# swoonge/SC-A-LOAM

Hardware: AMD Instinct MI355X
Metric: scans/sec (feat-extract + scan-to-map ICP + SC loop search), KITTI HDL-64 (higher is better)
Workload: dtype f32 points / f64 pose algebra

## Files before the change

### sc-a-loam_amd/csrc/common.hpp

```cpp
#pragma once
#include <hip/hip_runtime.h>
#include <hip/hip_ext.h>
#include <cstdio>
#include <cstdarg>
#include <cstring>
#include <string>
#include <vector>
#include <utility>
#include <mutex>
#include "../../include/scaloam_hip.h"
#include "batch.hpp"

namespace scal {
constexpr unsigned EV_DEVICE_ONLY = hipEventDisableTiming | hipEventDisableSystemFence;


void set_error(const char* fmt, ...);

#define SCAL_HIP(expr)                                                                         \
    do {                                                                                       \
        hipError_t _e = (expr);                                                                \
        if (_e != hipSuccess) {                                                                \
            ::scal::set_error("%s failed: %s (%s:%d)", #expr, hipGetErrorString(_e), __FILE__, __LINE__); \
            return SCAL_E_HIP;                                                                 \
        }                                                                                      \
    } while (0)

#define SCAL_TRY(expr)           \
    do {                         \
        int _rc = (expr);        \
        if (_rc != SCAL_OK) return _rc; \
    } while (0)

int select_device(int device);
enum class StreamLayout { Shared, PerStage };
enum { STAGE_FEATURES = 0, STAGE_SC = 1, STAGE_ODOM = 3, STAGE_MAP = 4, STAGE_MAP_PREFETCH = 2, STAGE_SC_FILTER = 5 };
int stage_lane(StreamLayout layout, int stage);
StreamLayout default_stream_layout();
int acquire_stream(int device, hipStream_t* out, int lane = 0);
void release_stream(int device, int lane = 0);
int odom_create(const scal_odom_config* cfg, StreamLayout layout, scal_odom_t** out);
int map_create(const scal_map_config* cfg, StreamLayout layout, scal_map_t** out);
int sc_create(const scal_sc_config* cfg, StreamLayout layout, scal_sc_t** out);
int icp_create_on_lane(const scal_icp_config* cfg, int lane, scal_icp_t** out);
int refine_create_on_lane(const scal_refine_config* cfg, int lane, scal_refine_t** out);
int posegraph_create_on_lane(const scal_posegraph_config* cfg, int lane, scal_posegraph_t** out);
struct ScFilterOut {
    const float *x, *y, *z, *w;
    const int* d_n;
    int cap;
};
int sc_insert_features_then(scal_sc_t* ctx, scal_features_t* feat, int (*after)(void* user, hipStream_t s, const ScFilterOut& ds), void* user);

int sc_make_cloud_device(scal_sc_t* ctx, const float* d_x, const float* d_y, const float* d_z, const int* d_n, int n_max, double* d_desc);

struct LaneStream {
    hipStream_t s = nullptr;
    int device = 0, lane = 0;
    LaneStream() = default;
    LaneStream(LaneStream&& o) noexcept { *this = std::move(o); }
    LaneStream& operator=(LaneStream&& o) noexcept {
        release();
        std::swap(s, o.s);
        device = o.device, lane = o.lane;
        return *this;
    }
    ~LaneStream() { release(); }
    operator hipStream_t() const { return s; }
    int acquire(int dev, int ln) {
        release();
        device = dev, lane = ln;
        return acquire_stream(dev, &s, ln);
    }
    void release() {
        if (s) release_stream(device, lane);
        s = nullptr;
// ... 147 lines not shown
```

### sc-a-loam_amd/csrc/mapping.hip

```cpp
#include "common.hpp"
#include <mutex>
#include <atomic>
#include "device_utils.hpp"
#include "voxel_dev.hpp"
#include "radix_sort.hpp"
#include "lm_host.hpp"
#include "features_dev.hpp"
#include <cmath>
#include <cstdlib>
#include <algorithm>
#include <deque>

namespace scal {

constexpr int CW = 21, CH = 21, CD = 11;
constexpr int GX = 250, GY = 250, GZ = 150;
constexpr int GCELLS = GX * GY * GZ;
constexpr unsigned long long MAP_NOMERGE = 127ull;

struct MapParams {
    int cenW, cenH, cenD;
    int cI, cJ, cK;
    int ox, oy, oz;
    float inv_line, inv_plane;
// ... 1089 lines not shown
__device__ __forceinline__ void k_merge_write_body(const MergeArgs& a, MapState* S, MapCounters* C, const MergeTail& t) {
    merge_write_body(a, S, C);
    if (!t.fused) return;
    if (static_cast<int>(blockIdx.x) >= MERGE_WRITE_GRID && S->pose_seq == t.seq) {
        const int i = (blockIdx.x - MERGE_WRITE_GRID) * 256 + threadIdx.x;
        if (i < min(*t.d_nfull, t.full_cap)) {
            double x7[7];
#pragma unroll
            for (int k = 0; k < 7; ++k) x7[k] = t.st->x[k];
            float sel[3];
            associate_to_map(x7, t.full.x[i], t.full.y[i], t.full.z[i], sel);
            t.full_out.x[i] = sel[0], t.full_out.y[i] = sel[1], t.full_out.z[i] = sel[2], t.full_out.w[i] = t.full.w[i];
        }
    }
}
SCAL_KERNEL(256, k_merge_write)

__device__ __forceinline__ void k_transform_cloud_body(const CSoA4& in, const int* __restrict__ d_n, int cap, const LMState* __restrict__ st,
                                                         const MapState* __restrict__ S, const SoA4& out) {
    if (S->abort) return;
    const int i = blockIdx.x * blockDim.x + threadIdx.x;
    if (i >= min(*d_n, cap)) return;
    double x7[7];
#pragma unroll
    for (int k = 0; k < 7; ++k) x7[k] = st->x[k];
    float sel[3];
    associate_to_map(x7, in.x[i], in.y[i], in.z[i], sel);
    out.x[i] = sel[0], out.y[i] = sel[1], out.z[i] = sel[2], out.w[i] = in.w[i];
}
SCAL_KERNEL(256, k_transform_cloud)

__device__ __forceinline__ void k_map_gather_body(const float* __restrict__ less_aos, const int* __restrict__ d_n_less, const CSoA4& less_flat,
                                                    const int* __restrict__ d_n_less_flat, const SoA4& corner_in, const SoA4& surf_in, MapCounters* C, int cap,
                                                    int nbc, unsigned* surf_parts) {
    const bool corner = static_cast<int>(blockIdx.x) < nbc;
    const int b = corner ? blockIdx.x : blockIdx.x - nbc;
    const int n = min(corner ? *d_n_less : *d_n_less_flat, cap);
    const int i = b * 256 + threadIdx.x;
    if (blockIdx.x == 0) {
        int* w = reinterpret_cast<int*>(C);
        for (int t = 2 + threadIdx.x; t < static_cast<int>(sizeof(MapCounters) / sizeof(int)); t += 256) w[t] = 0;
    }
    if (i == 0) (corner ? C->n_corner_in : C->n_surf_in) = n;
    if (corner) {
        if (i >= n) return;
        const float4 p = reinterpret_cast<const float4*>(less_aos)[i];
        corner_in.x[i] = p.x, corner_in.y[i] = p.y, corner_in.z[i] = p.z, corner_in.w[i] = p.w;
    } else {
        float x = 0.f, y = 0.f, z = 0.f;
        if (i < n) {
            x = less_flat.x[i], y = less_flat.y[i], z = less_flat.z[i];
            surf_in.x[i] = x, surf_in.y[i] = y, surf_in.z[i] = z, surf_in.w[i] = less_flat.w[i];
        }
        if (surf_parts) vox_bbox_block_store(surf_parts, b, i < n, x, y, z);
    }
}
SCAL_KERNEL(256, k_map_gather)

__device__ __forceinline__ void k_export_valid_body(const MapCloud& m, const MapState* __restrict__ S, int cls, int* __restrict__ counter,
                                                      float* __restrict__ out, int cap) {
    const MapParams mp = S->mp;
    const int n = S->n_map[cls];
    for (int i = blockIdx.x * blockDim.x + threadIdx.x; i < n; i += gridDim.x * blockDim.x)
        if (cube_valid(mp, m.cube[i])) {
            const int p = atomicAdd(counter, 1);
            if (p < cap) reinterpret_cast<float4*>(out)[p] = make_float4(m.x[i], m.y[i], m.z[i], m.w[i]);
        }
}
SCAL_KERNEL(256, k_export_valid)


__device__ __forceinline__ void copy_words(void* dst, const void* src, int bytes) {
    const unsigned* s = static_cast<const unsigned*>(src);
    unsigned* d = static_cast<unsigned*>(dst);
    for (int i = threadIdx.x; i < bytes / 4; i += blockDim.x) d[i] = s[i];
}

struct PoseDoneNew {
    CSoA4 stack[2];
    const int* d_ns[2];
// ... 97 lines not shown
using namespace scal;

int voxels_per_cell_axis(float leaf) {
    const double inv = 1.0 / static_cast<double>(leaf);
    int most = 1;
    for (int c = 0; c < 1000; ++c) {
        const int lo = static_cast<int>(std::floor(c * inv + 1e-4)), hi = static_cast<int>(std::floor((c + 1) * inv - 1e-4));
        most = std::max(most, hi - lo + 1);
    }
    return most;
}


struct MapStep {
    scal_features_t* feat = nullptr;
    MapPoseIn pose{};
    int set = 0;
    int slot = 0;
    int par = 0;
    bool prefetched = false, have_full = false, fast = false;
    bool pose_collected = false;
    bool confirmed = false;
    bool failed = false;
    bool prebuilt = false;
    unsigned seq = 0;
    unsigned feat_generation = 0;
    int n_corner_bound = 0, n_surf_bound = 0;
    int insert_path = 0;
};

struct InputSet {
    SoAStore in[2], stack[2];
    DevBuf<MapCounters> C;
    DevBuf<unsigned> surf_parts;
    Event ev_pre;
    Event ev_pre_a;
    int* n_in(int k) const { return k == 0 ? &C.p->n_corner_in : &C.p->n_surf_in; }
    int* n_stack(int k) const { return k == 0 ? &C.p->n_corner_stack : &C.p->n_surf_stack; }
};

template <class T, int N>
struct Fifo {
    T item[N];
    int n = 0;
    void push(const T& v) { item[n++] = v; }
    const T& front() const { return item[0]; }
    void pop() { std::copy(item + 1, item + n, item), --n; }
    void clear() { n = 0; }
};

struct scal_map {
    scal_map_config cfg;
    LaneStream stream;
    LaneStream side;
    static constexpr int NSETS = 8;
    static constexpr int MAX_STEPS = 4;
    static constexpr int MAX_PF = 3;
    static constexpr int NSLOTS = MAX_STEPS + 1;
    struct Prefetch {
        scal_features_t* feat;
        int set;
        unsigned generation;
    };
    std::mutex pf_mu;
    Fifo<Prefetch, MAX_PF> pf_half;
    Fifo<Prefetch, MAX_PF> pf;
    int next_set = 0;
// ... 45 lines not shown
    DevBuf<int> d_nfull;
    PinBuf<MapCounters> h_C;
    PinBuf<MapState> h_S;
    PinBuf<int> h_misc;
    int alloc_set() {
        const int st = next_set;
        next_set = (next_set + 1) % NSETS;
        return st;
    }
};

int scal::map_create(const scal_map_config* cfg, StreamLayout layout, scal_map_t** out) {
    if (!cfg || !out || cfg->max_scan_points <= 0 || cfg->max_map_points <= 0 || !(cfg->line_res > 0) || !(cfg->plane_res > 0)) {
        set_error("scal_map_create: bad argument");
        return SCAL_E_ARG;
    }
    if (cfg->line_res < 0.11f || cfg->plane_res < 0.11f) {
        set_error("mapping resolutions below 0.11 m exceed the 512 voxel/cube key layout");
        return SCAL_E_ARG;
    }
    *out = nullptr;
    SCAL_TRY(select_device(cfg->device));
    auto* c = new scal_map();
    c->cfg = *cfg;
    c->scan_cap = cfg->max_scan_points;
    c->map_cap = cfg->max_map_points;
    int rc = SCAL_OK;
    auto A = [&](int r) { if (rc == SCAL_OK) rc = r; };
    const size_t sc = c->scan_cap, mc = c->map_cap;
    A(c->aos.alloc(sc * 4));
    for (InputSet& I : c->sets) {
        A(I.in[0].alloc(sc)); A(I.in[1].alloc(sc)); A(I.stack[0].alloc(sc)); A(I.stack[1].alloc(sc));
        A(I.C.alloc(1));
        A(I.surf_parts.alloc((size_t)6 * (div_up(c->scan_cap, 256) + 1)));
    }
    A(c->full_in.alloc(sc)); A(c->full_out.alloc(sc));
    A(c->vf.init(c->scan_cap));
    A(c->vf_side.init(c->scan_cap));
    A(c->vf_corner.init(c->scan_cap));
    c->vf.set_tag(".C"), c->vf_side.set_tag(".C"), c->vf_corner.set_tag(".C");
    for (int k = 0; k < 2; ++k) {
        for (int b = 0; b < 2; ++b) {
            A(c->map[k].pts[b].alloc(mc));
            A(c->map[k].cube[b].alloc(mc));
        }
        for (int par = 0; par < 2; ++par) { A(c->grid[k].cell[par].alloc(GCELLS)); A(c->grid[k].rank[par].alloc(mc)); A(c->grid[k].okeys[par].alloc(mc)); }
        A(c->grid[k].g.alloc(mc));
    }
    A(c->sorter.init(c->map_cap));
    A(c->keys.alloc(mc)); A(c->vals.alloc(mc)); A(c->blockcnt.alloc(div_up(c->map_cap, 256) + 1));
    for (int k = 0; k < 2; ++k) {
        A(c->mnew[k].alloc(MERGE_MAX)); A(c->mcube[k].alloc(MERGE_MAX)); A(c->mpre[k].alloc(MERGE_MAX + 1)); A(c->mlb[k].alloc(MERGE_MAX));
        A(c->msorted[k].alloc(MERGE_MAX)); A(c->mhm[k].alloc(MERGE_MAX)); A(c->mblocktot[k].alloc(MERGE_CHUNKS));
        A(c->mpkey[k].alloc(MERGE_MAX)); A(c->msamp[k].alloc(MERGE_MAX / 8));
    }
    A(c->lm.alloc(c->scan_cap));
    A(c->nnrec.alloc(16 * sc));
    A(c->d_S.alloc(1)); A(c->d_nfull.alloc(4));
    A(c->blocks.alloc(c->scan_cap));
    A(c->h_C.alloc(1)); A(c->h_S.alloc(1)); A(c->h_misc.alloc(4)); A(c->res.alloc(scal_map::NSLOTS));
    const char* fixed_env = std::getenv("SCALOAM_MAP_FIXED_GRID");
    if (rc == SCAL_OK && !(fixed_env && fixed_env[0] == '0')) {
        int cap[2];
        for (int k = 0; k < 2; ++k) {
            const int a = voxels_per_cell_axis(c->leaf(k));
            cap[k] = a * a * a;
        }
// ... 27 lines not shown
        MapState& H = *c->h_S.p;
        std::memset(&H, 0, sizeof H);
        H.q_wmap_wodom[3] = 1.0;
        H.mp.cenW = 10, H.mp.cenH = 10, H.mp.cenD = 5;
        if (rc == SCAL_OK && op_memcpy_async(c->d_S.p, c->h_S.p, sizeof(MapState), hipMemcpyHostToDevice, c->stream) != hipSuccess) rc = SCAL_E_HIP;
        if (rc == SCAL_OK && op_stream_synchronize(c->stream) != hipSuccess) rc = SCAL_E_HIP;
    }
    if (rc != SCAL_OK) {
        if (rc == SCAL_E_HIP) set_error("scal_map_create: HIP resource creation failed");
        delete c;
        return rc;
    }
    *out = c;
    return SCAL_OK;
}

extern "C" int scal_map_create(const scal_map_config* cfg, scal_map_t** out) { return map_create(cfg, default_stream_layout(), out); }

extern "C" void scal_map_destroy(scal_map_t* c) {
    if (!c) return;
    (void)hipSetDevice(c->cfg.device);
    if (c->stream) (void)op_stream_synchronize(c->stream);
    if (c->side) (void)op_stream_synchronize(c->side);
    delete c;
}

namespace {

void copy_pose(double* q, double* t, const double* q_from, const double* t_from) {
    std::copy(q_from, q_from + 4, q);
    std::copy(t_from, t_from + 3, t);
}

int enqueue_stack_filter(scal_map* c, int k, VoxelFilter& vf, hipStream_t s, int n_bound, int st, bool surf_box_done = false) {
    InputSet& I = c->sets[st];
    VoxTail t;
    t.err_out = &I.C.p->error;
    const int bits = c->leaf(k) >= 0.35f ? 30 : 40;
    const bool box = k == 1 && surf_box_done && n_bound > 8192;
    return vf.run(s, I.in[k].cv(), I.n_in(k), n_bound, c->leaf(k), bits, I.stack[k].v(), I.n_stack(k), &t, box ? I.surf_parts.p : nullptr,
                  box ? std::max(1, div_up(n_bound, 256)) : 0);
}

GridArgs grid_args(scal_map* c, int par, bool fixed_pool = false) {
    GridArgs ga;
    for (int k = 0; k < 2; ++k) {
        GridStore& G = c->grid[k];
        ga.m[k] = c->map[k].cloud(par);
        ga.cell[k] = G.cell[par].p, ga.rank[k] = G.rank[par].p, ga.g[k] = G.pts(par, fixed_pool);
        ga.okeys[k] = G.okeys[par].p;
        ga.inv_leaf[k] = c->inv_leaf(k);
    }
    return ga;
}

int insert_full_sort(scal_map* c, const MapStep& e, const int* n_map) {
    hipStream_t s = c->stream;
    const InputSet& I = c->sets[e.set];
    MapCounters* C = I.C.p;
    LMState* st = c->lm.d_st.p;
    for (int k = 0; k < 2; ++k) {
        MapStore& M = c->map[k];
        const int n_tot_max = std::min(c->map_cap, n_map[k] + c->scan_cap);
        const int nb = std::max(1, div_up(n_tot_max, 256));
        MapCloud in = M.cloud(e.par), outc = M.cloud(e.par ^ 1);
        SCAL_LAUNCH("k_insert_keys", k_insert_keys, dim3(nb), dim3(256), 0, s, in, c->d_S.p, I.stack[k].cv(), I.n_stack(k), st, c->inv_leaf(k),
                           c->map_cap, c->keys.p, c->vals.p, C, k);
        SortedPairs sp;
        SCAL_TRY(c->sorter.sort(s, c->keys.p, c->vals.p, &C->n_total[k], n_tot_max, 36, nullptr, &sp));
        SCAL_LAUNCH("k_map_heads", k_map_heads, dim3(nb), dim3(256), 0, s, sp, &C->n_total[k], c->blockcnt.p);
        launch_scan_inplace(s, c->blockcnt.p, &C->n_total[k], 256, 1, &C->n_map_new[k]);
        SCAL_LAUNCH("k_map_reduce", k_map_reduce, dim3(nb), dim3(256), 0, s, sp, &C->n_total[k], c->blockcnt.p, in, outc);
    }
    SCAL_HIP(hipGetLastError());
// ... 77 lines not shown
}

MapPoseDone make_pose_done(scal_map* c, const MapStep& e) {
    const InputSet& I = c->sets[e.set];
    MapPoseDone pd;
    pd.active = 1, pd.seq = e.seq;
    pd.S = c->d_S.p, pd.st = c->lm.d_st.p, pd.C = I.C.p, pd.host = c->res.p + e.slot;
    for (int k = 0; k < 2; ++k) {
        pd.nw.stack[k] = I.stack[k].cv();
        pd.nw.d_ns[k] = I.n_stack(k);
        pd.nw.inv_leaf[k] = c->inv_leaf(k);
        pd.nw.x[k] = c->mnew[k].x.p, pd.nw.y[k] = c->mnew[k].y.p, pd.nw.z[k] = c->mnew[k].z.p, pd.nw.w[k] = c->mnew[k].w.p;
        pd.nw.cube[k] = c->mcube[k].p, pd.nw.pkey[k] = c->mpkey[k].p;
    }
    return pd;
}

int launch_pose_part(scal_map* c, const MapStep& e, bool prepare_only = false) {
    hipStream_t s = c->stream;
    const int st_ = e.set;
    InputSet& I = c->sets[st_];
    MapCounters* C = I.C.p;
    LMState* st = c->lm.d_st.p;
    MapState* S = c->d_S.p;
    if (e.feat) {
        if (e.prefetched) {
            SCAL_HIP(op_stream_wait_event(s, I.ev_pre, 0));
        } else {
            FeatDeviceView v = features_view(e.feat);
            SCAL_TRY(features_wait_done(e.feat, s));
            const int nbc = std::max(1, div_up(e.n_corner_bound, 256));
            SCAL_LAUNCH("k_map_gather", k_map_gather, dim3(nbc + std::max(1, div_up(e.n_surf_bound, 256))), dim3(256), 0, s, v.less_xyzi, &v.P->n_less_sharp,
                               CSoA4{v.lfx, v.lfy, v.lfz, v.lfi}, &v.P->n_less_flat, I.in[0].v(), I.in[1].v(), C, c->scan_cap, nbc,
                               static_cast<unsigned*>(nullptr));
        }
    }
    if (!e.prefetched) {
        SCAL_TRY(enqueue_stack_filter(c, 0, c->vf, s, e.n_corner_bound, st_));
        SCAL_TRY(enqueue_stack_filter(c, 1, c->vf, s, e.n_surf_bound, st_));
    }
    MapBeginArgs mb;
    mb.active = 0, mb.in = e.pose, mb.allow_window_change = e.fast ? 0 : 1, mb.inv_line = c->inv_leaf(0), mb.inv_plane = c->inv_leaf(1);
    mb.slot_cap = c->lm.slot_cap, mb.prebuilt = e.prebuilt ? 1 : 0, mb.S = S;
    const bool begin_in_knn = e.fast && e.prebuilt && c->grid_fixed && !prepare_only;
    if (!begin_in_knn) SCAL_LAUNCH("k_map_begin", k_map_begin, dim3(1), dim3(64), 0, s, mb, st, C);
    const bool fixed_pool = e.fast && c->grid_fixed && !prepare_only;
    const GridArgs ga = grid_args(c, e.par, fixed_pool);
    if (fixed_pool) {
        if (!e.prebuilt) SCAL_LAUNCH("k_grid_build", k_grid_build, dim3(GRID_BLOCKS), dim3(256), 0, s, ga, c->grid_cap_now[0], c->grid_cap_now[1], S, C);
    } else {
        SCAL_LAUNCH("k_grid_count", k_grid_count, dim3(GRID_BLOCKS), dim3(256), 0, s, ga, S, C);
        SCAL_LAUNCH("k_grid_alloc", k_grid_alloc, dim3(GRID_BLOCKS), dim3(256), 0, s, ga, S, C);
        SCAL_LAUNCH("k_grid_fill", k_grid_fill, dim3(GRID_BLOCKS), dim3(256), 0, s, ga, S);
    }
    if (prepare_only) {
        SCAL_HIP(hipGetLastError());
        return SCAL_OK;
    }
    FactorSoA F = c->lm.factors();
    const int assoc_blocks = std::max(1, std::min(3072, div_up(c->lm.slot_cap, 8)));
    MapPoseDone pd = make_pose_done(c, e);
    const AssocFit fit{I.stack[0].cv(), I.stack[1].cv(), c->nnbuf(), C, F};
    for (int outer = 0; outer < 2; ++outer) {
        {
            mb.active = (begin_in_knn && outer == 0) ? 1 : 0;
            SCAL_LAUNCH(mb.active ? "k_assoc_knn.0" : "k_assoc_knn", k_assoc_knn, dim3(assoc_blocks), dim3(256), 0, s, I.stack[0].cv(), I.stack[1].cv(), S,
                             c->grid[0].cell[e.par].p, c->grid[0].pts(e.par, fixed_pool), c->grid[1].cell[e.par].p, c->grid[1].pts(e.par, fixed_pool), st, C, c->nnbuf(), mb);
// ... 449 lines not shown
    SCAL_TRY(begin_sync_step(c, false, "scal_map_step: a queued step has not been collected", &e));
    SCAL_TRY(upload_step_inputs(c, e, corner_last, n_corner, surf_last, n_surf, full_res, have_full ? n_full : 0));
    copy_pose(e.pose.q_wodom, e.pose.t_wodom, q_wodom, t_wodom);
    SCAL_TRY(run_general_and_confirm(c, e));
    SCAL_TRY(map_collect_pose(c, q_w_curr, t_w_curr, stats));
    SCAL_TRY(map_settle(c, true));
    stats_after_insertion(c, stats);
    if (have_full && registered) SCAL_TRY(download_registered(c, registered, n_full));
    return SCAL_OK;
}

extern "C" int scal_map_prefetch_begin(scal_map_t* c, scal_features_t* feat) {
    if (!c || !feat) {
        set_error("scal_map_prefetch_begin: null argument");
        return SCAL_E_ARG;
    }
    FeatDeviceView v = features_view(feat);
    SCAL_TRY(check_features_device(c, v));
    SCAL_HIP(hipSetDevice(c->cfg.device));
    const int ls_cap = std::min(c->scan_cap, v.n_scans * 120);
    const int cap = std::min(c->scan_cap, v.cap);
    std::lock_guard<std::mutex> lk(c->pf_mu);
    if (c->pf.n + c->pf_half.n >= scal_map::MAX_PF) {
        set_error("scal_map_prefetch_features: %d prefetches are already queued ahead of their steps", scal_map::MAX_PF);
        return SCAL_E_STATE;
    }
    const int nset = c->alloc_set();
    InputSet& I = c->sets[nset];
    SCAL_TRY(I.ev_pre.ensure(EV_DEVICE_ONLY));
    SCAL_TRY(I.ev_pre_a.ensure(EV_DEVICE_ONLY));
    hipStream_t sa = v.stream;
    const int nbc = std::max(1, div_up(ls_cap, 256));
    SCAL_LAUNCH("k_map_gather", k_map_gather, dim3(nbc + std::max(1, div_up(cap, 256))), dim3(256), 0, sa, v.less_xyzi, &v.P->n_less_sharp,
                     CSoA4{v.lfx, v.lfy, v.lfz, v.lfi}, &v.P->n_less_flat, I.in[0].v(), I.in[1].v(), I.C.p, c->scan_cap, nbc, I.surf_parts.p);
    SCAL_HIP(hipGetLastError());
    SCAL_TRY(enqueue_stack_filter(c, 0, c->vf_corner, sa, ls_cap, nset));
    SCAL_HIP(op_event_record(I.ev_pre_a, sa));
    c->pf_half.push(scal_map::Prefetch{feat, nset, v.generation});
    return SCAL_OK;
}

extern "C" int scal_map_prefetch_finish(scal_map_t* c, scal_features_t* feat) {
    if (!c || !feat) {
        set_error("scal_map_prefetch_finish: null argument");
        return SCAL_E_ARG;
    }
    SCAL_HIP(hipSetDevice(c->cfg.device));
    FeatDeviceView v = features_view(feat);
    const int cap = std::min(c->scan_cap, v.cap);
    std::lock_guard<std::mutex> lk(c->pf_mu);
    if (c->pf_half.n == 0 || c->pf_half.front().feat != feat) {
        set_error("scal_map_prefetch_finish: no scal_map_prefetch_begin of this features context is waiting (halves are finished in the order they were begun)");
        return SCAL_E_STATE;
    }
    const scal_map::Prefetch h = c->pf_half.front();
    c->pf_half.pop();
    InputSet& I = c->sets[h.set];
    SCAL_HIP(op_stream_wait_event(c->side, I.ev_pre_a, 0));
    SCAL_TRY(enqueue_stack_filter(c, 1, c->vf_side, c->side, cap, h.set, true));
    SCAL_HIP(op_event_record(I.ev_pre, c->side));
    c->pf.push(h);
    return SCAL_OK;
}

extern "C" int scal_map_prefetch_features(scal_map_t* c, scal_features_t* feat) {
    SCAL_TRY(scal_map_prefetch_begin(c, feat));
    return scal_map_prefetch_finish(c, feat);
}

static int map_enqueue_features(scal_map* c, scal_features_t* feat, const double* q_wodom, const double* t_wodom) {
    FeatDeviceView v = features_view(feat);
    SCAL_TRY(check_features_device(c, v));
    SCAL_HIP(hipSetDevice(c->cfg.device));
    SCAL_TRY(map_make_room(c));
    MapStep e = new_step(c);
    e.feat = feat;
    e.feat_generation = v.generation;
    e.n_corner_bound = std::min(c->scan_cap, v.n_scans * 120);
    e.n_surf_bound = std::min(c->scan_cap, v.cap);
    e.have_full = true;
    copy_pose(e.pose.q_wodom, e.pose.t_wodom, q_wodom, t_wodom);
    {
        std::lock_guard<std::mutex> lk(c->pf_mu);
        if (c->pf.n > 0 && c->pf.front().feat == feat) {
            if (c->pf.front().generation != v.generation) {
                drop_prefetches(c);
                set_error("scal_map_enqueue_features: the features context was run again between scal_map_prefetch_features and this call");
                return SCAL_E_STATE;
            }
            e.prefetched = true;
            e.set = c->pf.front().set;
            c->pf.pop();
        } else {
            drop_prefetches(c);
// ... 234 lines not shown
```

### sc-a-loam_amd/csrc/pipeline.cpp

```cpp
#include "common.hpp"
#include "keyframes.hpp"
#include <algorithm>
#include <cmath>
#include <condition_variable>
#include <deque>
#include <chrono>
#include <cstdlib>
#include <string>
#include <thread>

namespace scal {
void print_forced_flushes();
}
using namespace scal;

namespace {
constexpr int REC_N = 64;
constexpr int MAX_UNPOPPED = 32;
constexpr int MAX_LOOPS_UNPOPPED = 64;
int env_int(const char* name, int dflt, int lo, int hi) {
    const char* e = std::getenv(name);
    if (!e) return dflt;
    const int v = std::atoi(e);
    return v < lo ? lo : (v > hi ? hi : v);
// ... 139 lines not shown
        if (st == SCAL_OK) {
            lk.lock();
            p->a_run = k + 1;
            p->cv.notify_all();
            lk.unlock();
            st = p->tm_front.run(1, "C: prefetch, lane 0 half", [&] { return p->for_all([&](int q) { return scal_map_prefetch_begin(p->mp[q], p->regs[q][slot]); }); });
        }
        lk.lock();
        if (st != SCAL_OK) {
            p->fail(st);
            return;
        }
        p->a_done = k + 1;
        p->cv.notify_all();
    }
}

void side_thread(scal_pipeline* p) {
    std::unique_lock<std::mutex> lk(p->mu);
    const bool search = p->cfg.sc_mode == SCAL_PIPE_SC_EVERY_SCAN;
    for (;;) {
        const long long k = p->pf_done;
        p->cv.wait(lk, [&] {
            if (p->stop || p->err) return true;
            if (p->a_done <= k) return false;
            return !(p->side_sc() && k - p->d_coll >= 3);
        });
        if (p->stop || p->err) return;
        const int slot = static_cast<int>(k % p->ring);
        lk.unlock();
        double* dd = p->d_desc ? p->d_desc + static_cast<size_t>(slot) * 1200 : nullptr;
        int st = p->tm_side.run(1, "C: prefetch, side half + D: insert", [&]() -> int {
            if (!p->side_sc() && p->S == 1) return scal_map_prefetch_finish(p->mp[0], p->regs[0][slot]);
            Recorder recs[2 * SMAX];
            Recorder* ptr[2 * SMAX];
            int nr = 0, rc2 = SCAL_OK;
            rc2 = p->tm_side.run(3, "   record prefetch", [&] {
                int r3 = SCAL_OK;
                for (int q = 0; q < p->S && r3 == SCAL_OK; ++q) {
                    g_recorder = ptr[nr] = &recs[nr];
                    ++nr;
                    r3 = scal_map_prefetch_finish(p->mp[q], p->regs[q][slot]);
                    g_recorder = nullptr;
                }
                return r3;
            });
            if (rc2 == SCAL_OK && p->side_sc())
                rc2 = p->tm_side.run(4, "   record insert", [&] {
                    int r3 = SCAL_OK;
                    for (int q = 0; q < p->S && r3 == SCAL_OK; ++q) {
                        g_recorder = ptr[nr] = &recs[nr];
                        ++nr;
                        r3 = search ? scal_sc_insert_features(p->sc[q], p->regs[q][slot]) : scal_sc_make_features_enqueue(p->sc[q], p->regs[q][slot], dd);
                        g_recorder = nullptr;
                    }
                    return r3;
                });
            if (rc2 != SCAL_OK) {
                for (int i = 0; i < nr; ++i) (void)recs[i].flush();
                return rc2;
            }
            return p->tm_side.run(5, "   zip + launch", [&]() -> int {
                if (zip_marked_and_launch(ptr, nr) != hipSuccess) {
                    set_error("scal_pipeline: a batched launch failed: %s", hipGetErrorString(hipGetLastError()));
                    return SCAL_E_HIP;
                }
                return SCAL_OK;
            });
        });
        if (st == SCAL_OK && search) st = p->tm_side.run(2, "D: sc_detect_enqueue", [&] { return p->for_all([&](int q) { return scal_sc_detect_enqueue(p->sc[q]); }); });
        lk.lock();
        if (st != SCAL_OK) {
            p->fail(st);
            return;
        }
        p->r(k).res[0].d_descriptor = dd;
        p->pf_done = k + 1;
        if (p->side_sc()) p->d_ins = k + 1;
        p->cv.notify_all();
    }
}

void odom_thread(scal_pipeline* p) {
    std::unique_lock<std::mutex> lk(p->mu);
    for (;;) {
        enum { NONE, B_ENQ, B_COLL } what = NONE;
        p->cv.wait(lk, [&] {
            if (p->stop || p->err) return true;
            if (p->b_enq < p->a_run && p->b_enq - p->b_coll < B_AHEAD) { what = B_ENQ; return true; }
            if (p->b_coll < p->b_enq && p->b_coll - p->c_enq < 2) { what = B_COLL; return true; }
            return false;
        });
        if (p->stop || p->err) return;
        int st = SCAL_OK;
        if (what == B_ENQ) {
            const long long k = p->b_enq;
// ... 660 lines not shown
```

### sc-a-loam_amd/csrc/voxel.hip

```cpp
#include "voxel_dev.hpp"
#include "device_utils.hpp"

namespace scal {

__device__ __forceinline__ void k_vox_bbox_body(const CSoA4& in, const int* __restrict__ d_n, unsigned* __restrict__ parts) {
    __shared__ unsigned s_lo[3][4], s_hi[3][4];
    const int n = *d_n;
    unsigned lo[3] = {0xffffffffu, 0xffffffffu, 0xffffffffu}, hi[3] = {0u, 0u, 0u};
    for (int i = blockIdx.x * blockDim.x + threadIdx.x; i < n; i += gridDim.x * blockDim.x) {
        const unsigned a = float_to_ordered(in.x[i]), b = float_to_ordered(in.y[i]), c = float_to_ordered(in.z[i]);
        lo[0] = min(lo[0], a), hi[0] = max(hi[0], a);
        lo[1] = min(lo[1], b), hi[1] = max(hi[1], b);
        lo[2] = min(lo[2], c), hi[2] = max(hi[2], c);
    }
#pragma unroll
    for (int a = 0; a < 3; ++a) {
#pragma unroll
        for (int o = 32; o > 0; o >>= 1) {
            lo[a] = min(lo[a], static_cast<unsigned>(__shfl_xor(static_cast<int>(lo[a]), o, 64)));
            hi[a] = max(hi[a], static_cast<unsigned>(__shfl_xor(static_cast<int>(hi[a]), o, 64)));
        }
        if (lane_id() == 0) s_lo[a][wave_id()] = lo[a], s_hi[a][wave_id()] = hi[a];
    }
    __syncthreads();
// ... 301 lines not shown
    while (t < lim && skey[t] == k) {
        ax += sx[t], ay += sy[t], az += sz[t], aw += sw[t];
        ++t;
    }
    int u = base + t;
    if (t == SPAN) {
        while (u < n && (sorted[u] >> 14) == k) {
            const int g = static_cast<int>(sorted[u] & 0x3fffu);
            ax += in.x[g], ay += in.y[g], az += in.z[g], aw += in.w[g];
            ++u;
        }
    }
    const float c = static_cast<float>(u - i);
    const int o = block_off + rank;
    out.x[o] = ax / c, out.y[o] = ay / c, out.z[o] = az / c, out.w[o] = aw / c;
}
SCAL_KERNEL(256, k_vox_small_reduce)
SCAL_DEFINE_STAMP_READER(scal_debug_stamps_voxel)

int VoxelFilter::init(int capacity) {
    cap = capacity;
    SCAL_TRY(sorter.init(cap));
    SCAL_TRY(keys.alloc(cap));
    SCAL_TRY(vals.alloc(cap));
    SCAL_TRY(blockcnt.alloc(div_up(cap, 256) + 1));
    SCAL_TRY(meta.alloc(1));
    SCAL_TRY(box_parts.alloc(6 * 128));
    SCAL_HIP(hipFuncSetAttribute(reinterpret_cast<const void*>(k_vox_small_sort), hipFuncAttributeMaxDynamicSharedMemorySize,
                                 static_cast<int>(sizeof(unsigned long long) * VOX_SMALL)));
    return SCAL_OK;
}

int VoxelFilter::run(hipStream_t s, CSoA4 in, const int* d_n, int n_bound, float leaf, int max_bits, SoA4 out, int* d_n_out, const VoxTail* tail,
                     const unsigned* ext_parts, int n_parts) {
    const float inv = 1.0f / leaf;
    const VoxTail tl = tail ? *tail : VoxTail();
    if (n_bound <= VOX_SMALL) {
        const int lds = sizeof(unsigned long long) * VOX_SMALL;
        const int n_cap = min(VOX_SMALL, cap);
        const int chunks = max(1, div_up(min(n_bound, n_cap), 512));
        SCAL_LAUNCH(n_small.c_str(), k_vox_small_sort, dim3(chunks), dim3(1024), lds, s, in, d_n, n_cap, inv, keys.p, meta.p, tl);
        SCAL_LAUNCH(n_small_reduce.c_str(), k_vox_small_reduce, dim3(max(1, div_up(min(n_bound, n_cap), 256))), dim3(256), 0, s, keys.p, d_n, n_cap, in, out,
                         d_n_out, tl);
        SCAL_HIP(hipGetLastError());
        return SCAL_OK;
    }
    const int nb = max(1, div_up(min(cap, n_bound), 256));
    if (!ext_parts) {
        n_parts = min(nb, 128);
        ext_parts = box_parts.p;
        SCAL_LAUNCH(n_bbox.c_str(), k_vox_bbox, dim3(n_parts), dim3(256), 0, s, in, d_n, box_parts.p);
    }
    rec_mark(true);
    SCAL_LAUNCH(n_keys.c_str(), k_vox_keys, dim3(nb), dim3(256), 0, s, in, d_n, inv, max_bits, meta.p, keys.p, vals.p, ext_parts, n_parts);
    SortedPairs sp;
    SCAL_TRY(sorter.sort(s, keys.p, vals.p, d_n, n_bound, max_bits, &meta.p->used_bits, &sp));
    SCAL_LAUNCH(n_heads.c_str(), k_vox_heads, dim3(nb), dim3(256), 0, s, sp, d_n, blockcnt.p);
    SCAL_LAUNCH(n_reduce.c_str(), k_vox_reduce, dim3(nb), dim3(256), 0, s, sp, d_n, blockcnt.p, in, out, d_n_out, meta.p, tl);
    rec_mark(false);
    SCAL_HIP(hipGetLastError());
    return SCAL_OK;
}

__device__ __forceinline__ void k_deinterleave_body(const float* __restrict__ aos, int n, const SoA4& o) {
    const int i = blockIdx.x * blockDim.x + threadIdx.x;
    if (i < n) {
        const float4 p = reinterpret_cast<const float4*>(aos)[i];
        o.x[i] = p.x, o.y[i] = p.y, o.z[i] = p.z, o.w[i] = p.w;
    }
}
// ... 91 lines not shown
    std::lock_guard<std::mutex> lk(c->mu);
    SCAL_HIP(hipSetDevice(c->device));
    hipStream_t s = c->stream;
    const float* d_in = xyzi;
    if (!on_device) {
        (void)c->hs.reserve((size_t)c->cap * 16 + 4096);
        SCAL_HIP(c->hs.h2d(c->aos.p, xyzi, sizeof(float) * 4 * n, s));
        d_in = c->aos.p;
    }
    SCAL_TRY(c->cf.load(s, d_in, n));
    SCAL_TRY(c->cf.filter(s, n, leaf));
    c->cf.store(s, n, on_device ? out_xyzi : c->aos.p);
    const int m = c->cf.wait(s, "scal_voxel_downsample");
    c->hs.finish();
    if (m < 0) return m;
    if (!on_device) {
        SCAL_HIP(c->hs.d2h(out_xyzi, c->aos.p, sizeof(float) * 4 * m, s));
        SCAL_HIP(op_stream_synchronize(s));
        c->hs.finish();
    }
    *n_out = m;
    return SCAL_OK;
}

extern "C" int scal_voxel_downsample(scal_voxel_t* c, const float* xyzi, int n, float leaf, float* out_xyzi, int* n_out) {
    return voxel_downsample(c, xyzi, n, leaf, out_xyzi, n_out, false);
}

extern "C" int scal_voxel_downsample_device(scal_voxel_t* c, const float* d_xyzi, int n, float leaf, float* d_out_xyzi, int* n_out) {
    return voxel_downsample(c, d_xyzi, n, leaf, d_out_xyzi, n_out, true);
}

extern "C" void* scal_voxel_stream(scal_voxel_t* c) { return c ? static_cast<void*>(c->stream) : nullptr; }
```

### sc-a-loam_amd/csrc/voxel_dev.hpp

```cpp
#pragma once
#include "common.hpp"
#include "radix_sort.hpp"

namespace scal {

struct VoxMeta {
    int error;
    int n_out;
    int guard;
    int used_bits;
    int b0, b1;
};

struct CSoA4 {
    const float *x, *y, *z, *w;
};
struct SoA4 {
    float *x, *y, *z, *w;
    operator CSoA4() const { return CSoA4{x, y, z, w}; }
};

struct VoxTail {
    int* err_out = nullptr;
    int* slots_out = nullptr;
    const int* other_n = nullptr;
    int slots_cap = 0;
};

struct VoxelFilter {
    int cap = 0;
    RadixSort sorter;
    DevBuf<unsigned long long> keys;
    DevBuf<int> vals;
    DevBuf<int> blockcnt;
    DevBuf<VoxMeta> meta;
    DevBuf<unsigned> box_parts;
    std::string n_bbox = "k_vox_bbox", n_keys = "k_vox_keys", n_heads = "k_vox_heads", n_reduce = "k_vox_reduce", n_small = "k_vox_small",
                n_small_reduce = "k_vox_small_reduce";
    void set_tag(const char* tag) {
        n_bbox = std::string("k_vox_bbox") + tag, n_keys = std::string("k_vox_keys") + tag, n_heads = std::string("k_vox_heads") + tag;
        n_reduce = std::string("k_vox_reduce") + tag, n_small = std::string("k_vox_small") + tag;
        n_small_reduce = std::string("k_vox_small_reduce") + tag;
        sorter.set_tag(tag);
    }

    int init(int capacity);
    int run(hipStream_t s, CSoA4 in, const int* d_n, int n_bound, float leaf, int max_bits, SoA4 out, int* d_n_out, const VoxTail* tail = nullptr,
            const unsigned* ext_parts = nullptr, int n_parts = 0);
};

void launch_deinterleave(hipStream_t s, const float* aos, int n, SoA4 o);
void launch_interleave(hipStream_t s, const int* d_n, int n_cap, CSoA4 in, float* aos);

struct CloudFilter {
    struct Host {
        int n_in, n_out;
        VoxMeta meta;
    };
    VoxelFilter vf;
    DevBuf<float> plane_in[4], plane_out[4];
    DevBuf<int> d_n;
    PinBuf<Host> h;

    int init(int capacity);
    bool ready() const { return h.p != nullptr; }
    void set_tag(const char* tag) { vf.set_tag(tag); }
    SoA4 in() const { return SoA4{plane_in[0].p, plane_in[1].p, plane_in[2].p, plane_in[3].p}; }
    SoA4 out() const { return SoA4{plane_out[0].p, plane_out[1].p, plane_out[2].p, plane_out[3].p}; }
    int* d_n_in() const { return d_n.p; }
    int* d_n_out() const { return d_n.p + 1; }
    int load(hipStream_t s, const float* d_xyzi, int n);
    void load_counted(hipStream_t s, const float* d_xyzi, int n) { launch_deinterleave(s, d_xyzi, n, in()); }
    int filter(hipStream_t s, int n, float leaf, const unsigned* ext_parts = nullptr, int n_parts = 0) {
        return vf.run(s, in(), d_n.p, n, leaf, 45, out(), d_n.p + 1, nullptr, ext_parts, n_parts);
    }
    void store(hipStream_t s, int n, float* d_xyzi) { launch_interleave(s, d_n.p + 1, n, out(), d_xyzi); }
    int wait(hipStream_t s, const char* who);
};

}

namespace scal {
#ifdef __HIPCC__
__device__ inline void vox_bbox_block_store(unsigned* parts, int block, unsigned lo[3], unsigned hi[3]) {
    __shared__ unsigned s_box[4][6];
#pragma unroll
    for (int a = 0; a < 3; ++a) {
#pragma unroll
        for (int o = 32; o > 0; o >>= 1) {
            lo[a] = min(lo[a], static_cast<unsigned>(__shfl_xor(static_cast<int>(lo[a]), o, 64)));
            hi[a] = max(hi[a], static_cast<unsigned>(__shfl_xor(static_cast<int>(hi[a]), o, 64)));
        }
        if ((threadIdx.x & 63) == 0) s_box[threadIdx.x >> 6][a] = lo[a], s_box[threadIdx.x >> 6][3 + a] = hi[a];
    }
    __syncthreads();
    if (threadIdx.x < 3)
        parts[block * 6 + threadIdx.x] = min(min(s_box[0][threadIdx.x], s_box[1][threadIdx.x]), min(s_box[2][threadIdx.x], s_box[3][threadIdx.x]));
    else if (threadIdx.x < 6)
        parts[block * 6 + threadIdx.x] = max(max(s_box[0][threadIdx.x], s_box[1][threadIdx.x]), max(s_box[2][threadIdx.x], s_box[3][threadIdx.x]));
}
__device__ __forceinline__ unsigned vox_ordered(float f) {
    const unsigned u = __float_as_uint(f);
    return (u & 0x80000000u) ? ~u : (u | 0x80000000u);
}
__device__ inline void vox_bbox_block_store(unsigned* parts, int block, bool have, float x, float y, float z) {
    unsigned lo[3] = {0xffffffffu, 0xffffffffu, 0xffffffffu}, hi[3] = {0u, 0u, 0u};
    if (have) {
// ... 9 lines not shown
```

Measured before the change: 4517.

## Move corner voxel filter to side stream and zip corner/surf launches together

The gather kernel now also computes per-block bounding boxes for corner points. The corner voxel filter moves from the prefetch stream to the side-stream finish step, where it runs on the general path with external bbox parts and a shared shape bound. Corner and surf filter launches are recorded into separate recorders, and their kernels are interleaved with the SC insert launches in a batched zip. The goal is to shorten the critical path on the main stream and let the two filters overlap. Forcing the general path and a shared shape bound may add work for small corner sets, and the corner key width changes from 40 to 36 bits in some configurations.

```diff
diff --git a/sc-a-loam_amd/csrc/common.hpp b/sc-a-loam_amd/csrc/common.hpp
--- a/sc-a-loam_amd/csrc/common.hpp
+++ b/sc-a-loam_amd/csrc/common.hpp
@@ -42,6 +42,7 @@
 int odom_create(const scal_odom_config* cfg, StreamLayout layout, scal_odom_t** out);
 int map_create(const scal_map_config* cfg, StreamLayout layout, scal_map_t** out);
 int sc_create(const scal_sc_config* cfg, StreamLayout layout, scal_sc_t** out);
+int map_prefetch_finish_lists(scal_map_t* ctx, scal_features_t* feat, Recorder* corner, Recorder* surf);
 int icp_create_on_lane(const scal_icp_config* cfg, int lane, scal_icp_t** out);
 int refine_create_on_lane(const scal_refine_config* cfg, int lane, scal_refine_t** out);
 int posegraph_create_on_lane(const scal_posegraph_config* cfg, int lane, scal_posegraph_t** out);
diff --git a/sc-a-loam_amd/csrc/mapping.hip b/sc-a-loam_amd/csrc/mapping.hip
--- a/sc-a-loam_amd/csrc/mapping.hip
+++ b/sc-a-loam_amd/csrc/mapping.hip
@@ -1145,7 +1145,7 @@
 
 __device__ __forceinline__ void k_map_gather_body(const float* __restrict__ less_aos, const int* __restrict__ d_n_less, const CSoA4& less_flat,
                                                     const int* __restrict__ d_n_less_flat, const SoA4& corner_in, const SoA4& surf_in, MapCounters* C, int cap,
-                                                    int nbc, unsigned* surf_parts) {
+                                                    int nbc, unsigned* surf_parts, unsigned* corner_parts) {
     const bool corner = static_cast<int>(blockIdx.x) < nbc;
     const int b = corner ? blockIdx.x : blockIdx.x - nbc;
     const int n = min(corner ? *d_n_less : *d_n_less_flat, cap);
@@ -1156,9 +1156,12 @@
     }
     if (i == 0) (corner ? C->n_corner_in : C->n_surf_in) = n;
     if (corner) {
-        if (i >= n) return;
-        const float4 p = reinterpret_cast<const float4*>(less_aos)[i];
-        corner_in.x[i] = p.x, corner_in.y[i] = p.y, corner_in.z[i] = p.z, corner_in.w[i] = p.w;
+        float4 p = make_float4(0.f, 0.f, 0.f, 0.f);
+        if (i < n) {
+            p = reinterpret_cast<const float4*>(less_aos)[i];
+            corner_in.x[i] = p.x, corner_in.y[i] = p.y, corner_in.z[i] = p.z, corner_in.w[i] = p.w;
+        }
+        if (corner_parts) vox_bbox_block_store(corner_parts, b, i < n, p.x, p.y, p.z);
     } else {
         float x = 0.f, y = 0.f, z = 0.f;
         if (i < n) {
@@ -1322,7 +1325,7 @@
 struct InputSet {
     SoAStore in[2], stack[2];
     DevBuf<MapCounters> C;
-    DevBuf<unsigned> surf_parts;
+    DevBuf<unsigned> parts[2];
     Event ev_pre;
     Event ev_pre_a;
     int* n_in(int k) const { return k == 0 ? &C.p->n_corner_in : &C.p->n_surf_in; }
@@ -1434,7 +1437,7 @@
     for (InputSet& I : c->sets) {
         A(I.in[0].alloc(sc)); A(I.in[1].alloc(sc)); A(I.stack[0].alloc(sc)); A(I.stack[1].alloc(sc));
         A(I.C.alloc(1));
-        A(I.surf_parts.alloc((size_t)6 * (div_up(c->scan_cap, 256) + 1)));
+        for (int k = 0; k < 2; ++k) A(I.parts[k].alloc((size_t)6 * (div_up(c->scan_cap, 256) + 1)));
     }
     A(c->full_in.alloc(sc)); A(c->full_out.alloc(sc));
     A(c->vf.init(c->scan_cap));
@@ -1528,14 +1531,22 @@
     std::copy(t_from, t_from + 3, t);
 }
 
-int enqueue_stack_filter(scal_map* c, int k, VoxelFilter& vf, hipStream_t s, int n_bound, int st, bool surf_box_done = false) {
+int enqueue_stack_filter(scal_map* c, int k, VoxelFilter& vf, hipStream_t s, int n_bound, int st) {
     InputSet& I = c->sets[st];
     VoxTail t;
     t.err_out = &I.C.p->error;
     const int bits = c->leaf(k) >= 0.35f ? 30 : 40;
-    const bool box = k == 1 && surf_box_done && n_bound > 8192;
-    return vf.run(s, I.in[k].cv(), I.n_in(k), n_bound, c->leaf(k), bits, I.stack[k].v(), I.n_stack(k), &t, box ? I.surf_parts.p : nullptr,
-                  box ? std::max(1, div_up(n_bound, 256)) : 0);
+    return vf.run(s, I.in[k].cv(), I.n_in(k), n_bound, c->leaf(k), bits, I.stack[k].v(), I.n_stack(k), &t);
+}
+
+int enqueue_stack_filter_shared(scal_map* c, int k, VoxelFilter& vf, hipStream_t s, int shape_bound, int n_parts, int st) {
+    InputSet& I = c->sets[st];
+    VoxTail t;
+    t.err_out = &I.C.p->error;
+    int bits = c->leaf(k) >= 0.35f ? 30 : 40;
+    if (k == 0 && bits == 40 && c->leaf(1) >= 0.35f) bits = 36;
+    return vf.run(s, I.in[k].cv(), I.n_in(k), shape_bound, c->leaf(k), bits, I.stack[k].v(), I.n_stack(k), &t, I.parts[k].p, n_parts,
+                  VoxelFilter::Path::General);
 }
 
 GridArgs grid_args(scal_map* c, int par, bool fixed_pool = false) {
@@ -1679,7 +1690,7 @@
             const int nbc = std::max(1, div_up(e.n_corner_bound, 256));
             SCAL_LAUNCH("k_map_gather", k_map_gather, dim3(nbc + std::max(1, div_up(e.n_surf_bound, 256))), dim3(256), 0, s, v.less_xyzi, &v.P->n_less_sharp,
                                CSoA4{v.lfx, v.lfy, v.lfz, v.lfi}, &v.P->n_less_flat, I.in[0].v(), I.in[1].v(), C, c->scan_cap, nbc,
-                               static_cast<unsigned*>(nullptr));
+                               static_cast<unsigned*>(nullptr), static_cast<unsigned*>(nullptr));
         }
     }
     if (!e.prefetched) {
@@ -2195,21 +2206,31 @@
     hipStream_t sa = v.stream;
     const int nbc = std::max(1, div_up(ls_cap, 256));
     SCAL_LAUNCH("k_map_gather", k_map_gather, dim3(nbc + std::max(1, div_up(cap, 256))), dim3(256), 0, sa, v.less_xyzi, &v.P->n_less_sharp,
-                     CSoA4{v.lfx, v.lfy, v.lfz, v.lfi}, &v.P->n_less_flat, I.in[0].v(), I.in[1].v(), I.C.p, c->scan_cap, nbc, I.surf_parts.p);
+                     CSoA4{v.lfx, v.lfy, v.lfz, v.lfi}, &v.P->n_less_flat, I.in[0].v(), I.in[1].v(), I.C.p, c->scan_cap, nbc, I.parts[1].p, I.parts[0].p);
     SCAL_HIP(hipGetLastError());
-    SCAL_TRY(enqueue_stack_filter(c, 0, c->vf_corner, sa, ls_cap, nset));
     SCAL_HIP(op_event_record(I.ev_pre_a, sa));
     c->pf_half.push(scal_map::Prefetch{feat, nset, v.generation});
     return SCAL_OK;
 }
 
-extern "C" int scal_map_prefetch_finish(scal_map_t* c, scal_features_t* feat) {
+namespace {
+struct RecorderScope {
+    Recorder* keep;
+    explicit RecorderScope(Recorder* r) : keep(g_recorder) {
+        if (r) g_recorder = r;
+    }
+    ~RecorderScope() { g_recorder = keep; }
+};
+}
+
+int scal::map_prefetch_finish_lists(scal_map_t* c, scal_features_t* feat, Recorder* corner, Recorder* surf) {
     if (!c || !feat) {
         set_error("scal_map_prefetch_finish: null argument");
         return SCAL_E_ARG;
     }
     SCAL_HIP(hipSetDevice(c->cfg.device));
     FeatDeviceView v = features_view(feat);
+    const int ls_cap = std::min(c->scan_cap, v.n_scans * 120);
     const int cap = std::min(c->scan_cap, v.cap);
     std::lock_guard<std::mutex> lk(c->pf_mu);
     if (c->pf_half.n == 0 || c->pf_half.front().feat != feat) {
@@ -2219,10 +2240,34 @@
     const scal_map::Prefetch h = c->pf_half.front();
     c->pf_half.pop();
     InputSet& I = c->sets[h.set];
-    SCAL_HIP(op_stream_wait_event(c->side, I.ev_pre_a, 0));
-    SCAL_TRY(enqueue_stack_filter(c, 1, c->vf_side, c->side, cap, h.set, true));
-    SCAL_HIP(op_event_record(I.ev_pre, c->side));
+    const int shape = std::max(cap, ls_cap);
+    {
+        RecorderScope rs(corner);
+        SCAL_HIP(op_stream_wait_event(c->side, I.ev_pre_a, 0));
+        SCAL_TRY(enqueue_stack_filter_shared(c, 0, c->vf_corner, c->side, shape, std::max(1, div_up(ls_cap, 256)), h.set));
+    }
+    {
+        RecorderScope rs(surf);
+        SCAL_TRY(enqueue_stack_filter_shared(c, 1, c->vf_side, c->side, shape, std::max(1, div_up(cap, 256)), h.set));
+        SCAL_HIP(op_event_record(I.ev_pre, c->side));
+    }
     c->pf.push(h);
+    return SCAL_OK;
+}
+
+extern "C" int scal_map_prefetch_finish(scal_map_t* c, scal_features_t* feat) {
+    if (g_recorder) return map_prefetch_finish_lists(c, feat, nullptr, nullptr);
+    Recorder recs[2];
+    Recorder* ptr[2] = {&recs[0], &recs[1]};
+    const int rc = map_prefetch_finish_lists(c, feat, ptr[0], ptr[1]);
+    if (rc != SCAL_OK) {
+        for (Recorder& r : recs) (void)r.flush();
+        return rc;
+    }
+    if (zip_marked_and_launch(ptr, 2) != hipSuccess) {
+        set_error("scal_map_prefetch_finish: a launch failed: %s", hipGetErrorString(hipGetLastError()));
+        return SCAL_E_HIP;
+    }
     return SCAL_OK;
 }
 
diff --git a/sc-a-loam_amd/csrc/pipeline.cpp b/sc-a-loam_amd/csrc/pipeline.cpp
--- a/sc-a-loam_amd/csrc/pipeline.cpp
+++ b/sc-a-loam_amd/csrc/pipeline.cpp
@@ -195,24 +195,22 @@
         double* dd = p->d_desc ? p->d_desc + static_cast<size_t>(slot) * 1200 : nullptr;
         int st = p->tm_side.run(1, "C: prefetch, side half + D: insert", [&]() -> int {
             if (!p->side_sc() && p->S == 1) return scal_map_prefetch_finish(p->mp[0], p->regs[0][slot]);
-            Recorder recs[2 * SMAX];
-            Recorder* ptr[2 * SMAX];
+            Recorder recs[3 * SMAX];
             int nr = 0, rc2 = SCAL_OK;
             rc2 = p->tm_side.run(3, "   record prefetch", [&] {
                 int r3 = SCAL_OK;
                 for (int q = 0; q < p->S && r3 == SCAL_OK; ++q) {
-                    g_recorder = ptr[nr] = &recs[nr];
-                    ++nr;
-                    r3 = scal_map_prefetch_finish(p->mp[q], p->regs[q][slot]);
-                    g_recorder = nullptr;
+                    nr += 2;
+                    r3 = map_prefetch_finish_lists(p->mp[q], p->regs[q][slot], &recs[nr - 2], &recs[nr - 1]);
                 }
                 return r3;
             });
-            if (rc2 == SCAL_OK && p->side_sc())
+            const int n_sc = (rc2 == SCAL_OK && p->side_sc()) ? p->S : 0;
+            if (n_sc)
                 rc2 = p->tm_side.run(4, "   record insert", [&] {
                     int r3 = SCAL_OK;
                     for (int q = 0; q < p->S && r3 == SCAL_OK; ++q) {
-                        g_recorder = ptr[nr] = &recs[nr];
+                        g_recorder = &recs[nr];
                         ++nr;
                         r3 = search ? scal_sc_insert_features(p->sc[q], p->regs[q][slot]) : scal_sc_make_features_enqueue(p->sc[q], p->regs[q][slot], dd);
                         g_recorder = nullptr;
@@ -223,8 +221,13 @@
                 for (int i = 0; i < nr; ++i) (void)recs[i].flush();
                 return rc2;
             }
+            Recorder* ptr[3 * SMAX];
+            int np = 0;
+            for (int q = 0; q < p->S; ++q) ptr[np++] = &recs[2 * q + 1];
+            for (int q = 0; q < n_sc; ++q) ptr[np++] = &recs[2 * p->S + q];
+            for (int q = 0; q < p->S; ++q) ptr[np++] = &recs[2 * q];
             return p->tm_side.run(5, "   zip + launch", [&]() -> int {
-                if (zip_marked_and_launch(ptr, nr) != hipSuccess) {
+                if (zip_marked_and_launch(ptr, np) != hipSuccess) {
                     set_error("scal_pipeline: a batched launch failed: %s", hipGetErrorString(hipGetLastError()));
                     return SCAL_E_HIP;
                 }
diff --git a/sc-a-loam_amd/csrc/voxel.hip b/sc-a-loam_amd/csrc/voxel.hip
--- a/sc-a-loam_amd/csrc/voxel.hip
+++ b/sc-a-loam_amd/csrc/voxel.hip
@@ -357,10 +357,14 @@
 }
 
 int VoxelFilter::run(hipStream_t s, CSoA4 in, const int* d_n, int n_bound, float leaf, int max_bits, SoA4 out, int* d_n_out, const VoxTail* tail,
-                     const unsigned* ext_parts, int n_parts) {
+                     const unsigned* ext_parts, int n_parts, Path path) {
     const float inv = 1.0f / leaf;
     const VoxTail tl = tail ? *tail : VoxTail();
-    if (n_bound <= VOX_SMALL) {
+    if (path == Path::Small && n_bound > VOX_SMALL) {
+        set_error("VoxelFilter::run: the small path takes at most %d points, the bound is %d", VOX_SMALL, n_bound);
+        return SCAL_E_ARG;
+    }
+    if (path != Path::General && n_bound <= VOX_SMALL) {
         const int lds = sizeof(unsigned long long) * VOX_SMALL;
         const int n_cap = min(VOX_SMALL, cap);
         const int chunks = max(1, div_up(min(n_bound, n_cap), 512));
@@ -518,3 +522,26 @@
 }
 
 extern "C" void* scal_voxel_stream(scal_voxel_t* c) { return c ? static_cast<void*>(c->stream) : nullptr; }
+
+extern "C" int scal_debug_voxel_path(scal_voxel_t* c, const float* d_xyzi, int n, int n_bound, float leaf, int path, float* d_out_xyzi, int* n_out) {
+    if (!c || !n_out || n < 0 || (n > 0 && (!d_xyzi || !d_out_xyzi)) || !(leaf > 0.f) || (path != 0 && path != 1)) {
+        set_error("scal_debug_voxel_path: bad argument");
+        return SCAL_E_ARG;
+    }
+    if (n_bound == 0) n_bound = n;
+    if (n > n_bound || n_bound > c->cap) {
+        set_error("scal_debug_voxel_path: %d points, bound %d, capacity %d", n, n_bound, c->cap);
+        return SCAL_E_TOO_MANY;
+    }
+    *n_out = 0;
+    std::lock_guard<std::mutex> lk(c->mu);
+    SCAL_HIP(hipSetDevice(c->device));
+    hipStream_t s = c->stream;
+    SCAL_TRY(c->cf.load(s, d_xyzi, n));
+    SCAL_TRY(c->cf.filter(s, n_bound, leaf, nullptr, 0, path == 0 ? VoxelFilter::Path::Small : VoxelFilter::Path::General));
+    c->cf.store(s, n, d_out_xyzi);
+    const int m = c->cf.wait(s, "scal_debug_voxel_path");
+    if (m < 0) return m;
+    *n_out = m;
+    return SCAL_OK;
+}
diff --git a/sc-a-loam_amd/csrc/voxel_dev.hpp b/sc-a-loam_amd/csrc/voxel_dev.hpp
--- a/sc-a-loam_amd/csrc/voxel_dev.hpp
+++ b/sc-a-loam_amd/csrc/voxel_dev.hpp
@@ -45,8 +45,9 @@
     }
 
     int init(int capacity);
+    enum class Path { Auto, Small, General };
     int run(hipStream_t s, CSoA4 in, const int* d_n, int n_bound, float leaf, int max_bits, SoA4 out, int* d_n_out, const VoxTail* tail = nullptr,
-            const unsigned* ext_parts = nullptr, int n_parts = 0);
+            const unsigned* ext_parts = nullptr, int n_parts = 0, Path path = Path::Auto);
 };
 
 void launch_deinterleave(hipStream_t s, const float* aos, int n, SoA4 o);
@@ -71,8 +72,8 @@
     int* d_n_out() const { return d_n.p + 1; }
     int load(hipStream_t s, const float* d_xyzi, int n);
     void load_counted(hipStream_t s, const float* d_xyzi, int n) { launch_deinterleave(s, d_xyzi, n, in()); }
-    int filter(hipStream_t s, int n, float leaf, const unsigned* ext_parts = nullptr, int n_parts = 0) {
-        return vf.run(s, in(), d_n.p, n, leaf, 45, out(), d_n.p + 1, nullptr, ext_parts, n_parts);
+    int filter(hipStream_t s, int n, float leaf, const unsigned* ext_parts = nullptr, int n_parts = 0, VoxelFilter::Path path = VoxelFilter::Path::Auto) {
+        return vf.run(s, in(), d_n.p, n, leaf, 45, out(), d_n.p + 1, nullptr, ext_parts, n_parts, path);
     }
     void store(hipStream_t s, int n, float* d_xyzi) { launch_interleave(s, d_n.p + 1, n, out(), d_xyzi); }
     int wait(hipStream_t s, const char* who);
```

After: 4427. 0.98x the previous value.
